# StanislavParovoy/VQ-VAE-WaveNet

Hardware: AMD Instinct MI355X
Metric: training audio-samples/sec (higher is better)
Workload: dtype f32 via fp16x3 (storage and accumulation fp32; the engine's contraction operands are each fp32 value split into two fp16 planes = 22-23 significand bits, products h1h1 + h1h2 + h2h1 on the fp16 MFMA, device-side range guards -- forward, input and weight gradients of the residual stack, of the 1x1 co; 1 GPU; VCTK '64' encoder, len=6656 batch=8 per GPU, fp32 (fp16x3 engine), full train step (fwd+bwd+allreduce+Adam+EMA); global_batch=8, seq_len=6656, parallelism=dp1

## Files before the change

vq-vae-wavenet_amd/csrc/gate_f16x3.hip:

```cpp
#include <string.h>

#include <type_traits>

#include "vqw_common.h"

namespace {

typedef _Float16 f16x8 __attribute__((ext_vector_type(8)));
typedef unsigned short u16;

typedef __bf16 bf16x8 __attribute__((ext_vector_type(8)));
__device__ __forceinline__ u16 f16_bits(_Float16 h) { return __builtin_bit_cast(u16, h); }
__device__ __forceinline__ u16 bf16_bits(float x) { return __builtin_bit_cast(u16, (__bf16)x); }
template <bool BF = false>
__device__ __forceinline__ void split8(const float (&x)[8], uint4& p0, uint4& p1) {
    u16 a[8], b[8];
#pragma unroll
    for (int e = 0; e < 8; ++e) {
        if (BF) { a[e] = bf16_bits(x[e]); b[e] = 0; continue; }
        float xe = x[e];
        asm volatile("" : "+v"(xe));
        const _Float16 h1 = (_Float16)xe;
        a[e] = f16_bits(h1);
        b[e] = f16_bits((_Float16)(xe - (float)h1));
    }
    p0 = make_uint4(a[0] | ((unsigned)a[1] << 16), a[2] | ((unsigned)a[3] << 16), a[4] | ((unsigned)a[5] << 16), a[6] | ((unsigned)a[7] << 16));
    p1 = make_uint4(b[0] | ((unsigned)b[1] << 16), b[2] | ((unsigned)b[3] << 16), b[4] | ((unsigned)b[5] << 16), b[6] | ((unsigned)b[7] << 16));
}

constexpr float F16_MAX = 65504.0f;
__device__ __forceinline__ float dev_scale(const float* p) { return p ? *p : 1.0f; }
__device__ __forceinline__ float inv_scales(float host_inv, const float* sa, const float* sb) {
    return (sa || sb) ? host_inv * __builtin_amdgcn_rcpf(dev_scale(sa) * dev_scale(sb)) : host_inv;
}
__device__ __forceinline__ float wave_max(float v) {
#pragma unroll
    for (int o = 32; o > 0; o >>= 1) v = fmaxf(v, __shfl_xor(v, o, 64));
    return v;
}
__device__ __forceinline__ void guard_report(float m, bool bad, float ps, unsigned* amax, int* flag) {
    if (!amax && !flag) return;
    const float wm = wave_max(m);
    const bool wbad = __any(bad || !(m * ps <= F16_MAX));
    if ((threadIdx.x & 63) == 0) {
        const unsigned bits = __float_as_uint(wm);
        if (amax && bits > __hip_atomic_load(amax, __ATOMIC_RELAXED, __HIP_MEMORY_SCOPE_AGENT)) atomicMax(amax, bits);
        if (flag && wbad) atomicOr(flag, 1);
    }
}

template <bool BF>
__global__ void split_act_kernel(const float* __restrict__ x, uint4* __restrict__ planes, int B, int C, int T, float scale, int kc0, int KC,
                                 const float* __restrict__ scale_dev, unsigned* amax, int* flag, int s2d) {
    const size_t NB = (size_t)B * T;
    const size_t i = (size_t)blockIdx.x * blockDim.x + threadIdx.x;
    const bool live = i < NB * (C / 8);
    const float sc = scale * dev_scale(scale_dev);
    float m = 0.0f;
    bool bad = false;
    if (live) {
        const size_t row = i % NB;
        const int kc = (int)(i / NB);
        const int b = (int)(row / T), t = (int)(row % T);
        float v[8];
#pragma unroll
        for (int e = 0; e < 8; ++e) {
            const float xv = x[((size_t)b * C + kc * 8 + e) * T + t];
            v[e] = xv * sc;
            bad |= !(fabsf(xv) <= 3.0e38f);
            m = fmaxf(m, fabsf(xv));
        }
        uint4 p0, p1;
        split8<BF>(v, p0, p1);
        if (s2d) {
            const size_t NH = NB / 2, r2 = (size_t)b * (T / 2) + t / 2;
            const int kcs = (t & 1) * (C / 8) + kc;
            planes[(size_t)kcs * NH + r2] = p0;
            if (!BF) planes[((size_t)(C / 4) + kcs) * NH + r2] = p1;
        } else {
            planes[(size_t)(kc0 + kc) * NB + row] = p0;
            if (!BF) planes[((size_t)KC + kc0 + kc) * NB + row] = p1;
        }
    }
    if (!amax && !flag) return;
    __shared__ float smax[4];
    __shared__ int sbad[4];
    const float wm = wave_max(m);
    const bool wbad = __any(bad || !(m * sc <= F16_MAX));
    if ((threadIdx.x & 63) == 0) { smax[threadIdx.x >> 6] = wm; sbad[threadIdx.x >> 6] = wbad; }
    __syncthreads();
    if (threadIdx.x == 0) {
        const unsigned bits = __float_as_uint(fmaxf(fmaxf(smax[0], smax[1]), fmaxf(smax[2], smax[3])));
        if (amax && bits > __hip_atomic_load(amax, __ATOMIC_RELAXED, __HIP_MEMORY_SCOPE_AGENT)) atomicMax(amax, bits);
        if (flag && (sbad[0] | sbad[1] | sbad[2] | sbad[3])) atomicOr(flag, 1);
    }
}

__global__ void amax_kernel(const float* __restrict__ x, long rows, int cols, long ld, long mstride, unsigned* amax, int* flag) {
    const float* xb = x + (size_t)blockIdx.y * mstride;
    const size_t n = (size_t)rows * cols;
    float m = 0.0f;
    bool bad = false;
    const size_t tid = (size_t)blockIdx.x * blockDim.x + threadIdx.x, nthr = (size_t)gridDim.x * blockDim.x;
    if (ld == cols && (n & 3) == 0 && (reinterpret_cast<uintptr_t>(xb) & 15u) == 0) {
        const f32x4* x4 = reinterpret_cast<const f32x4*>(xb);
        const size_t n4 = n >> 2;
        auto fold = [&](const f32x4 v) {
#pragma unroll
            for (int e = 0; e < 4; ++e) {
                const float a = fabsf(v[e]);
                bad |= !(a <= 3.0e38f);
                m = fmaxf(m, a);
            }
        };
        size_t i = tid;
        for (; i + 7 * nthr < n4; i += 8 * nthr) {
            f32x4 v[8];
#pragma unroll
            for (int u = 0; u < 8; ++u) v[u] = __builtin_nontemporal_load(x4 + i + u * nthr);
#pragma unroll
            for (int u = 0; u < 8; ++u) fold(v[u]);
        }
        for (; i < n4; i += nthr) fold(__builtin_nontemporal_load(x4 + i));
    } else {
        for (size_t i = tid; i < n; i += nthr) {
            const float v = xb[(i / cols) * ld + (i % cols)];
            bad |= !(fabsf(v) <= 3.0e38f);
            m = fmaxf(m, fabsf(v));
        }
    }
    __shared__ float smax[4];
    __shared__ int sbad[4];
    const float wm = wave_max(m);
    const bool wbad = __any(bad);
    if ((threadIdx.x & 63) == 0) { smax[threadIdx.x >> 6] = wm; sbad[threadIdx.x >> 6] = wbad; }
    __syncthreads();
    if (threadIdx.x == 0) {
        const unsigned bits = __float_as_uint(fmaxf(fmaxf(smax[0], smax[1]), fmaxf(smax[2], smax[3])));
        unsigned* dst = amax + blockIdx.y;
        if (bits > __hip_atomic_load(dst, __ATOMIC_RELAXED, __HIP_MEMORY_SCOPE_AGENT)) atomicMax(dst, bits);
        if (flag && (sbad[0] | sbad[1] | sbad[2] | sbad[3])) atomicOr(flag, 1);
    }
}

__global__ void update_scales_kernel(unsigned* amax, float* scale, int n, int target_exp, int reset, int* flag, const int* skip) {
    const int i = blockIdx.x * blockDim.x + threadIdx.x;
    if (i >= n || (skip && *skip)) return;
    const unsigned b = amax[i];
    if (b >= 0x7f800000u) {
        if (flag) atomicOr(flag, 1);
    } else if (b != 0) {
        int e = (int)(b >> 23) - 127;
        int se = target_exp - 1 - e;
        se = se > 100 ? 100 : (se < -100 ? -100 : se);
        scale[i] = __uint_as_float((unsigned)(se + 127) << 23);
    } else if (scale[i] == 0.0f) {
        scale[i] = 1.0f;
    }
    if (reset) amax[i] = 0;
}

template <bool BF>
__global__ void pack_gate_w_kernel(const float* __restrict__ w, uint4* __restrict__ planes, int ks, int R, int ldw, float scale,
                                   const float* __restrict__ scale_dev, int hb) {
    scale *= dev_scale(scale_dev);
    const int M = 2 * R, KC = ks * R / 8;
    w += (size_t)blockIdx.y * ks * R * ldw;
    planes += (size_t)blockIdx.y * 2 * KC * M;
    const int i = blockIdx.x * blockDim.x + threadIdx.x;
    if (i >= KC * M) return;
    const int mp = i % M, kc = i / M;
    const int mt = mp / hb, ii = mp % hb, hh = hb / 2;
    const int col = ii < hh ? hh * mt + ii : R + hh * mt + (ii - hh);
    const int j = kc / (R / 8), c0 = (kc % (R / 8)) * 8;
    float v[8];
#pragma unroll
    for (int e = 0; e < 8; ++e) v[e] = w[((size_t)j * R + c0 + e) * ldw + col] * scale;
    uint4 p0, p1;
    split8<BF>(v, p0, p1);
    planes[(size_t)kc * M + mp] = p0;
    if (!BF) planes[((size_t)KC + kc) * M + mp] = p1;
}

template <bool BF>
__global__ void pack_w_kernel(const float* __restrict__ w, uint4* __restrict__ planes, int K, int M, int ldw, float scale,
                              const float* __restrict__ scale_dev) {
    scale *= dev_scale(scale_dev);
    const int KC = K / 8;
    w += (size_t)blockIdx.y * K * ldw;
    planes += (size_t)blockIdx.y * 2 * KC * M;
    const int i = blockIdx.x * blockDim.x + threadIdx.x;
    if (i >= KC * M) return;
    const int m = i % M, kc = i / M;
    float v[8];
#pragma unroll
    for (int e = 0; e < 8; ++e) v[e] = w[(size_t)(kc * 8 + e) * ldw + m] * scale;
    uint4 p0, p1;
    split8<BF>(v, p0, p1);
    planes[(size_t)kc * M + m] = p0;
    if (!BF) planes[((size_t)KC + kc) * M + m] = p1;
}

template <bool BF>
__global__ void pack_w_t_kernel(const float* __restrict__ w, uint4* __restrict__ planes, int K, int M, int Kin, int ld_src, long blk_stride,
                                float scale, const float* __restrict__ scale_dev) {
    scale *= dev_scale(scale_dev);
    const int KC = K / 8;
    w += (size_t)blockIdx.y * (K / Kin) * blk_stride;
    planes += (size_t)blockIdx.y * 2 * KC * M;
    const int i = blockIdx.x * blockDim.x + threadIdx.x;
    if (i >= KC * M) return;
    const int m = i % M, kc = i / M, k0 = kc * 8, jb = k0 / Kin, ko = k0 - jb * Kin;
    const float* src = w + (size_t)jb * blk_stride + (size_t)m * ld_src + ko;
    const f32x4 a = *reinterpret_cast<const f32x4*>(src), b = *reinterpret_cast<const f32x4*>(src + 4);
    float v[8];
#pragma unroll
    for (int e = 0; e < 4; ++e) { v[e] = a[e] * scale; v[4 + e] = b[e] * scale; }
    uint4 p0, p1;
    split8<BF>(v, p0, p1);
    planes[(size_t)kc * M + m] = p0;
    if (!BF) planes[((size_t)KC + kc) * M + m] = p1;
}

template <bool BF>
__global__ __launch_bounds__(256) void pack_w_t_tile_kernel(const float* __restrict__ w, uint4* __restrict__ planes, int K, int M, int Kin, int ld_src,
                                                            long blk_stride, float scale, const float* __restrict__ scale_dev) {
    __shared__ uint4 lp[2][8][65];
    scale *= dev_scale(scale_dev);
    const int KC = K / 8, mt = (M + 63) / 64;
    const int m0 = (blockIdx.x % mt) * 64, kc0 = (blockIdx.x / mt) * 8, k0 = kc0 * 8, jb = k0 / Kin, ko0 = k0 - jb * Kin;
    w += (size_t)blockIdx.y * (K / Kin) * blk_stride + (size_t)jb * blk_stride + ko0;
    planes += (size_t)blockIdx.y * 2 * KC * M;
#pragma unroll
    for (int r = 0; r < 2; ++r) {
        const int e = threadIdx.x + 256 * r, mm = e >> 3, kq = e & 7;
        float v[8];
        if (m0 + mm < M) {
            const float* src = w + (size_t)(m0 + mm) * ld_src + kq * 8;
            const f32x4 a = *reinterpret_cast<const f32x4*>(src), b = *reinterpret_cast<const f32x4*>(src + 4);
#pragma unroll
            for (int i = 0; i < 4; ++i) { v[i] = a[i] * scale; v[4 + i] = b[i] * scale; }
        } else {
#pragma unroll
            for (int i = 0; i < 8; ++i) v[i] = 0.0f;
        }
        uint4 p0, p1;
        split8<BF>(v, p0, p1);
        lp[0][kq][mm] = p0;
        if (!BF) lp[1][kq][mm] = p1;
    }
    __syncthreads();
#pragma unroll
    for (int r = 0; r < 2; ++r) {
        const int e = threadIdx.x + 256 * r, kq = e >> 6, mm = e & 63;
        if (m0 + mm >= M) continue;
        planes[(size_t)(kc0 + kq) * M + m0 + mm] = lp[0][kq][mm];
        if (!BF) planes[((size_t)KC + kc0 + kq) * M + m0 + mm] = lp[1][kq][mm];
    }
}

struct GateArgs {
    vqw_f16x3_gate_desc d;
    int NB;
    int ratio;
};
struct OutArgs {
    vqw_f16x3_out_desc d;
    int NB;
};

#ifndef VQW_WG_PAT_A
#define VQW_WG_PAT_A 4
#define VQW_WG_PAT_B 2
#endif

#ifndef VQW_SCONV_64
#define VQW_SCONV_64 1
#endif
#ifndef VQW_SCONV_192
#define VQW_SCONV_192 1
#endif
#ifndef VQW_X3_TAP_MINOR
#define VQW_X3_TAP_MINOR 1
#endif
#ifndef VQW_X3_PAT_MEM
#define VQW_X3_PAT_MEM 1
#define VQW_X3_PAT_ALU 2
#endif
constexpr int NSTG = 4, STG_BYTES = 32 * 1024, PIECES = 8;

struct LoopGeom {
    const void* wp;
    const void* xp;
    int M, Cin, ks, dilation, NB, m_row0, n0, t0;
    int xKC, xkc0;
    int dir, T;
    int wks, tj0, tjstep, toff, tsgn, ts2d;
    int sb, sn;
};

#ifndef VQW_X3_STAGGER
#define VQW_X3_STAGGER 0
#endif
__device__ __forceinline__ void x3_stagger(int n) {
    if (VQW_X3_STAGGER > 0 && ((blockIdx.x >> 8) & 1))
        for (int i = 0; i < n; ++i) __builtin_amdgcn_s_sleep(127);
}
template <int MR> struct X3Shape {
    static constexpr int NSTAGE = MR == 8 ? 4 : 3;
    static constexpr int STAGE_BYTES = (MR * 2 + 16) * 1024;
    static constexpr int LDS_BYTES = NSTAGE * STAGE_BYTES;
    static constexpr int DEPTH = MR == 8 ? 2 : 1;
};
template <bool BF, int MR, bool TAB = false, int DEPTH = X3Shape<MR>::DEPTH>
__device__ __forceinline__ void f16x3_mainloop(f32x16 (&acc)[MR][2], char* smem, const LoopGeom& g, int wv, int lane) {
    constexpr int NP = BF ? 1 : 2;
    constexpr int NA = MR * NP / 4, NBP = 2 * NP;
    if (MR == 4) x3_stagger(VQW_X3_STAGGER);
    constexpr int NSTG_ = DEPTH + 2, STGB = X3Shape<MR>::STAGE_BYTES, BOFF = MR * 2 * 1024;
    const int l31 = lane & 31, lhi = lane >> 5;
    const int KCA = (TAB ? g.wks : g.ks) * g.Cin / 8, KCB = g.Cin / 8, spt = g.Cin / 16;
    const int nsteps = TAB ? g.sn : g.ks * spt;
    const __amdgpu_buffer_rsrc_t ra = vqw_make_rsrc(g.wp, (unsigned)((size_t)NP * KCA * g.M * 16));
    const size_t plane_bytes = (size_t)g.xKC * g.NB * 16, span = (size_t)(g.xKC - g.xkc0) * g.NB * 16;
    const char* xbase = reinterpret_cast<const char*>(g.xp) + (size_t)g.xkc0 * g.NB * 16;
    const unsigned xspan = span < 0x7fffffffu ? (unsigned)span : 0x7fffffffu;
    const __amdgpu_buffer_rsrc_t rb0 = vqw_make_rsrc(xbase, xspan);
    const __amdgpu_buffer_rsrc_t rb1 = vqw_make_rsrc(xbase + (NP > 1 ? plane_bytes : 0), xspan);
    int voffA[NA], pieceA[NA], voffB[NBP], trow[NBP], pieceB[NBP];
#pragma unroll
    for (int i = 0; i < NA; ++i) {
        const int q = wv * NA + i, tile = q / NP, p = q % NP;
        pieceA[i] = tile * 2 + p;
        voffA[i] = ((p * KCA + lhi) * g.M + g.m_row0 + tile * 32 + l31) * 16;
    }
#pragma unroll
    for (int i = 0; i < NBP; ++i) {
        const int q = wv * NBP + i, tile = q / NP, p = q % NP;
        pieceB[i] = tile * 2 + p;
        voffB[i] = (lhi * g.NB + g.n0 + tile * 32 + l31) * 16;
        trow[i] = TAB ? (g.n0 + tile * 32 + l31) % g.T : g.t0 + tile * 32 + l31;
    }
    f32x4 rgA[NA + NBP], rgB[NA + NBP];
    auto rissue = [&](int s_, f32x4 (&rg)[NA + NBP]) {
        const int s = TAB ? s_ + g.sb : s_;
#if VQW_X3_TAP_MINOR
        const int ji = TAB ? s / spt : s % g.ks, kc = TAB ? (s - ji * spt) * 2 : (s / g.ks) * 2;
#else
        const int ji = s / spt, kc = (s - ji * spt) * 2;
#endif
        const int j = TAB ? g.tj0 + g.tjstep * ji : ji;
        const int e_ = TAB ? j - g.toff : 0;
        const int shift = TAB ? g.tsgn * (e_ >> 1) : (g.ks - 1 - j) * g.dilation * (g.dir < 0 ? -1 : 1);
        const int kcx = TAB ? kc + (g.ts2d ? (e_ & 1) * KCB : 0) : kc;
#pragma unroll
        for (int i = 0; i < NA; ++i) rg[i] = vqw_buf_load4(ra, voffA[i] + (j * KCB + kc) * g.M * 16, 0);
#pragma unroll
        for (int i = 0; i < NBP; ++i) {
            const int tr = trow[i] - shift;
            const int vb = (tr >= 0 && tr < g.T) ? voffB[i] + (kcx * g.NB - shift) * 16 : (int)0x80000000;
            rg[NA + i] = vqw_buf_load4((i % NP) ? rb1 : rb0, vb, 0);
        }
    };
    auto rcommit = [&](int s, const f32x4 (&rg)[NA + NBP]) {
        char* dst = smem + (s % NSTG_) * STGB + lane * 16;
#pragma unroll
        for (int i = 0; i < NA; ++i) *reinterpret_cast<f32x4*>(dst + pieceA[i] * 1024) = rg[i];
#pragma unroll
        for (int i = 0; i < NBP; ++i) *reinterpret_cast<f32x4*>(dst + BOFF + pieceB[i] * 1024) = rg[NA + i];
    };
    uint4 fa[MR][NP], fb[2][NP], fbn[2][NP];
    auto read_a = [&](int i, int s) {
        const char* st = smem + (s % NSTG_) * STGB + lane * 16;
#pragma unroll
        for (int p = 0; p < NP; ++p) fa[i][p] = *reinterpret_cast<const uint4*>(st + (i * 2 + p) * 1024);
    };
    auto read_b = [&](uint4 (&b)[2][NP], int s) {
        const char* st = smem + (s % NSTG_) * STGB + lane * 16 + BOFF;
#pragma unroll
        for (int j = 0; j < 2; ++j)
#pragma unroll
            for (int p = 0; p < NP; ++p) b[j][p] = *reinterpret_cast<const uint4*>(st + ((wv * 2 + j) * 2 + p) * 1024);
    };
#pragma unroll
    for (int i = 0; i < MR; ++i)
#pragma unroll
        for (int j = 0; j < 2; ++j)
#pragma unroll
            for (int r = 0; r < 16; ++r) acc[i][j][r] = 0.f;
    auto mfma_rows = [&](int i, const uint4 (&b)[2][NP]) {
        if constexpr (BF) {
#pragma unroll
            for (int q = 0; q < 4; ++q)
                acc[i + (q >> 1)][q & 1] = __builtin_amdgcn_mfma_f32_32x32x16_bf16(__builtin_bit_cast(bf16x8, fa[i + (q >> 1)][0]), __builtin_bit_cast(bf16x8, b[q & 1][0]), acc[i + (q >> 1)][q & 1], 0, 0, 0);
        } else {
#pragma unroll
            for (int term = 0; term < 3; ++term)
#pragma unroll
                for (int q = 0; q < 4; ++q) {
                    const int ii = i + (q >> 1), j = q & 1;
                    const int pa = term == 1 ? 1 : 0, pb = term == 0 ? 1 : 0;
                    acc[ii][j] = __builtin_amdgcn_mfma_f32_32x32x16_f16(__builtin_bit_cast(f16x8, fa[ii][pa]), __builtin_bit_cast(f16x8, b[j][pb]), acc[ii][j], 0, 0, 0);
                }
        }
    };

    rissue(0, rgA); rcommit(0, rgA);
    rissue(1, rgA); rcommit(1, rgA);
    rissue(2, rgA);
    if (DEPTH == 2) rissue(3, rgB);
    asm volatile("s_waitcnt lgkmcnt(0)\n\ts_barrier" ::: "memory");
#pragma unroll
    for (int i = 0; i < MR; ++i) read_a(i, 0);
    read_b(fb, 0);
    auto step = [&](const uint4 (&bc)[2][NP], uint4 (&bn)[2][NP], int s, f32x4 (&rg)[NA + NBP]) {
        asm volatile("s_waitcnt lgkmcnt(0)\n\ts_barrier" ::: "memory");
        const int sn = s + 1 < nsteps ? s + 1 : s;
#ifndef VQW_ABL_NOLDSREAD
        read_b(bn, sn);
#endif
#ifndef VQW_ABL_NOCOMMIT
        rcommit(s + 2, rg);
#endif
#ifndef VQW_ABL_NOGLOBAL
        rissue(s + 2 + DEPTH, rg);
#endif
#pragma unroll
        for (int i = 0; i < MR; i += 2) {
            mfma_rows(i, bc);
#ifndef VQW_ABL_NOLDSREAD
            read_a(i, sn);
            read_a(i + 1, sn);
#endif
        }
#pragma unroll
        for (int k_ = 0; k_ < (BF ? 2 : 6) * MR; ++k_) {
            __builtin_amdgcn_sched_group_barrier(0x008, 1, 0);
            __builtin_amdgcn_sched_group_barrier(0x100 | 0x200 | 0x020, BF ? 2 : VQW_X3_PAT_MEM, 0);
            __builtin_amdgcn_sched_group_barrier(0x002 | 0x004, VQW_X3_PAT_ALU, 0);
        }
    };
    for (int s = 0; s < nsteps; s += 2) {
        step(fb, fbn, s, rgA);
        step(fbn, fb, s + 1, DEPTH == 2 ? rgB : rgA);
    }
}

template <int NG, int DEPTH, typename Ops, typename Req, typename Fin>
__device__ __forceinline__ void x3_epilogue_pipeline(Req&& request, Fin&& finish) {
    static_assert(NG % 2 == 0 && DEPTH >= 0 && DEPTH <= 2, "two named buffers");
    Ops p0, p1;
    request(0, p0);
    if constexpr (DEPTH == 0) {
#pragma unroll
        for (int g = 0; g < NG; ++g) {
            if (g > 0) request(g, p0);
            finish(g, p0);
        }
    } else if constexpr (DEPTH == 2) {
        request(1, p1);
#pragma unroll
        for (int g = 0; g < NG; g += 2) {
            { const Ops c = p0; if (g + 2 < NG) request(g + 2, p0); finish(g, c); }
                { const Ops c = p1; if (g + 3 < NG) request(g + 3, p1); finish(g + 1, c); }
            }
    } else {
#pragma unroll
        for (int g = 0; g < NG; g += 2) {
            request(g + 1, p1);
            finish(g, p0);
                if (g + 2 < NG) request(g + 2, p0);
            finish(g + 1, p1);
            }
    }
}
__device__ __forceinline__ unsigned x3_present(bool present) {
    unsigned m = __builtin_amdgcn_readfirstlane(present ? 0xffffffffu : 0u);
    asm volatile("" : "+s"(m));
    return m;
}
__device__ __forceinline__ float x3_masked(float v, unsigned m) { return __uint_as_float(__float_as_uint(v) & m); }
__device__ __forceinline__ int x3_masked(int i, unsigned m) { return (int)((unsigned)i & m); }
__device__ __forceinline__ void x3_pin_guard(float& gmax, bool& gbad) {
    int gb_i = (int)gbad;
    asm volatile("" : "+v"(gmax), "+v"(gb_i));
    gbad = gb_i != 0;
}
#ifndef VQW_X3_EPI_DEPTH
#define VQW_X3_EPI_DEPTH 2
#endif
#ifndef VQW_X3_GATE_EPI_DEPTH
#define VQW_X3_GATE_EPI_DEPTH 0
#endif
constexpr int EPI_DEPTH = VQW_X3_EPI_DEPTH;

template <bool BF>
__device__ __forceinline__ void store_plane_quad(void* planes, int KC, int NB, int kc, int row, int lhi, const float (&x)[4], float scale = 1.0f) {
    u16 h1[4], h2[4];
#pragma unroll
    for (int e = 0; e < 4; ++e) {
        const float xs = x[e] * scale;
        if (BF) { h1[e] = bf16_bits(xs); h2[e] = 0; continue; }
        const _Float16 a = (_Float16)xs;
        h1[e] = f16_bits(a);
        h2[e] = f16_bits((_Float16)(xs - (float)a));
    }
    char* base = reinterpret_cast<char*>(planes) + ((size_t)kc * NB + row) * 16 + lhi * 8;
    *reinterpret_cast<uint2*>(base) = make_uint2(h1[0] | ((unsigned)h1[1] << 16), h1[2] | ((unsigned)h1[3] << 16));
    if (!BF) *reinterpret_cast<uint2*>(base + (size_t)KC * NB * 16) = make_uint2(h2[0] | ((unsigned)h2[1] << 16), h2[2] | ((unsigned)h2[3] << 16));
}

template <bool BF, int MR>
__global__ __launch_bounds__(256, MR == 8 ? 1 : 2) void gate_f16x3_kernel(const GateArgs a) {
    extern __shared__ __attribute__((aligned(1024))) char smem[];
    const vqw_f16x3_gate_desc& d = a.d;
    const int tid = threadIdx.x, lane = tid & 63, wv = tid >> 6, l31 = lane & 31, lhi = lane >> 5;
    const int R = d.R, T = d.T;
    constexpr int HB = 32 * MR, HH = HB / 2;
    const int n_mt = R / HH;
    const int bid = vqw_xcd_remap(blockIdx.x, gridDim.x);
    const int mt = bid % n_mt, n0 = (bid / n_mt) * 256;
    const int b = n0 / T, t0 = n0 - b * T;
    f32x16 acc[MR][2];
    {
        LoopGeom g;
        g.wp = d.wp; g.xp = d.xp; g.M = 2 * R; g.Cin = R; g.ks = d.ks; g.dilation = d.dilation; g.NB = a.NB;
        g.xKC = R / 8; g.xkc0 = 0; g.dir = 1; g.T = T;
        g.m_row0 = mt * HB; g.n0 = n0; g.t0 = t0;
        f16x3_mainloop<BF, MR>(acc, smem, g, wv, lane);
    }

    const bool hb = d.bias != nullptr, hc = d.cond != nullptr;
    const float* bp = hb ? d.bias : reinterpret_cast<const float*>(d.wp);
    const float* cb = hc ? d.cond + (size_t)b * d.cond_bstride : reinterpret_cast<const float*>(d.wp);
    const int tcol = t0 + 64 * wv + l31;
    const int tz0 = (t0 + 64 * wv) / a.ratio, tz1 = (t0 + 64 * wv + 32) / a.ratio;
    const float winv = inv_scales(d.w_scale_inv, d.x_scale, d.w_scale);
    const unsigned mb = x3_present(hb), mc = x3_present(hc);
    struct Ops { float bf[4], bg[4], f0[4], f1[4], g0[4], g1[4]; };
    auto epilogue = [&](auto step_c) {
        constexpr bool STEP = decltype(step_c)::value;
        const bool s0 = STEP ? false : d.save0 != nullptr, s1 = STEP ? true : d.save1 != nullptr;
        const bool w0 = STEP ? false : d.out0 != nullptr, wp_ = STEP ? true : d.out_planes != nullptr;
        auto request = [&](int g, Ops& o) {
            const int i = g >> 2, v4 = g & 3;
            const int c0 = HH * mt + 32 * i + 8 * v4 + 4 * lhi;
#pragma unroll
            for (int e = 0; e < 4; ++e) {
                o.bf[e] = bp[x3_masked(c0 + e, mb)]; o.bg[e] = bp[x3_masked(R + c0 + e, mb)];
                const int cf = (c0 + e) * d.cond_T, cg = (R + c0 + e) * d.cond_T;
                o.f0[e] = cb[x3_masked(cf + tz0, mc)]; o.f1[e] = cb[x3_masked(cf + tz1, mc)];
                o.g0[e] = cb[x3_masked(cg + tz0, mc)]; o.g1[e] = cb[x3_masked(cg + tz1, mc)];
            }
        };
        auto finish = [&](int g, const Ops& o) {
            const int i = g >> 2, v4 = g & 3;
            const int c0 = HH * mt + 32 * i + 8 * v4 + 4 * lhi;
            float addf[4][2], addg[4][2];
#pragma unroll
            for (int e = 0; e < 4; ++e) {
                const float bfv = o.bf[e], bgv = o.bg[e], f0 = o.f0[e], f1 = o.f1[e], g0 = o.g0[e], g1 = o.g1[e];
                addf[e][0] = x3_masked(bfv, mb) + x3_masked(f0, mc); addf[e][1] = x3_masked(bfv, mb) + x3_masked(f1, mc);
                addg[e][0] = x3_masked(bgv, mb) + x3_masked(g0, mc); addg[e][1] = x3_masked(bgv, mb) + x3_masked(g1, mc);
            }
            const size_t off = ((size_t)b * R + c0) * T + tcol;
            float* po = (w0 ? d.out0 : d.save1) + off;
            float* p0 = s0 ? d.save0 + off : po;
            float* p1 = s1 ? d.save1 + off : po;
            float gq[2][4];
#pragma unroll
            for (int e = 0; e < 4; ++e)
#pragma unroll
                for (int j = 0; j < 2; ++j) {
                    const float xf = acc[i][j][v4 * 4 + e] * winv + addf[e][j];
                    const float xg = acc[i + MR / 2][j][v4 * 4 + e] * winv + addg[e][j];
                    const float th = 1.0f - 2.0f * __builtin_amdgcn_rcpf(__expf(2.0f * xf) + 1.0f);
                    const float sg = __builtin_amdgcn_rcpf(1.0f + __expf(-xg));
                    const int o_ = e * T + 32 * j;
                    gq[j][e] = th * sg;
                    if constexpr (STEP) asm volatile("" : "+v"(gq[j][e]));
                    if (s0) p0[o_] = th;
                    if (s1) p1[o_] = sg;
                    if (w0) po[o_] = gq[j][e];
                }
            if (wp_) {
#pragma unroll
                for (int j = 0; j < 2; ++j)
                    store_plane_quad<BF>(d.out_planes, d.out_planes_KC > 0 ? d.out_planes_KC : R / 8, a.NB, d.out_planes_kc0 + (HH / 8) * mt + 4 * i + v4,
                                     n0 + 64 * wv + 32 * j + l31, lhi, gq[j]);
            }
        };
        x3_epilogue_pipeline<MR * 2, VQW_X3_GATE_EPI_DEPTH, Ops>(request, finish);
    };
    if (!d.out0 && !d.save0 && d.save1 && d.out_planes) epilogue(std::true_type{});
    else epilogue(std::false_type{});
}

template <bool BF, int MR>
__global__ __launch_bounds__(256, MR == 8 ? 1 : 2) void out_f16x3_kernel(const OutArgs a) {
    extern __shared__ __attribute__((aligned(1024))) char smem[];
    const vqw_f16x3_out_desc& d = a.d;
    const int tid = threadIdx.x, lane = tid & 63, wv = tid >> 6, l31 = lane & 31, lhi = lane >> 5;
    const int R = d.R, S = d.S, T = d.T, M = S + R;
    const int Cin = d.Cin > 0 ? d.Cin : R;
    constexpr int HB = 32 * MR;
    const int n_mt = M / HB;
    const int bid = vqw_xcd_remap(blockIdx.x, gridDim.x);
    const int mt = bid % n_mt, n0 = (bid / n_mt) * 256;
    const int b = n0 / T, t0 = n0 - b * T;
    f32x16 acc[MR][2];
    {
        LoopGeom g;
        g.wp = d.wp; g.xp = d.xp; g.M = M; g.Cin = Cin; g.ks = d.ks > 0 ? d.ks : 1; g.dilation = d.dilation > 0 ? d.dilation : 1; g.NB = a.NB;
        g.xKC = d.xp_KC > 0 ? d.xp_KC : Cin / 8; g.xkc0 = d.xp_kc0; g.dir = d.dir < 0 ? -1 : 1; g.T = T;
        g.m_row0 = mt * HB; g.n0 = n0; g.t0 = t0;
        f16x3_mainloop<BF, MR>(acc, smem, g, wv, lane);
    }
    const bool is_skip = mt * HB < S;
    const bool hb = d.bias != nullptr;
    const float* bp = hb ? d.bias : reinterpret_cast<const float*>(d.wp);
    const int tcol = t0 + 64 * wv + l31;
    const float winv = inv_scales(d.w_scale_inv, d.x_scale, d.w_scale);
    const float ps = (d.plane_scale > 0.0f ? d.plane_scale : 1.0f) * dev_scale(d.out_scale);
    const bool hin = is_skip || d.net_in != nullptr;
    const unsigned mb = x3_present(hb), min_ = x3_present(hin);
    const float* in_base = is_skip ? d.skip : (d.net_in ? d.net_in : d.net_out);
    float* out_base = is_skip ? d.skip : d.net_out;
    const int nrows = is_skip ? S : R, mrow0 = is_skip ? 0 : S;
    struct Ops { float bq[4], old[2][4]; };
    auto epilogue = [&](auto pl_c) {
        constexpr bool PL = decltype(pl_c)::value;
        float gmax = 0.0f;
        bool gbad = false;
        auto offset = [&](int g, int& m0) {
            const int i = g >> 2, v4 = g & 3;
            m0 = mt * HB + 32 * i + 8 * v4 + 4 * lhi;
            return ((size_t)b * nrows + (m0 - mrow0)) * T + tcol;
        };
        auto request = [&](int g, Ops& o) {
            int m0;
            const size_t off = offset(g, m0);
            const float* pin = in_base + off;
#pragma unroll
            for (int e = 0; e < 4; ++e) {
                o.bq[e] = bp[x3_masked(m0 + e, mb)];
#pragma unroll
                for (int j = 0; j < 2; ++j) o.old[j][e] = pin[e * T + 32 * j];
            }
        };
        auto finish = [&](int g, const Ops& o) {
            const int i = g >> 2, v4 = g & 3;
            int m0;
            const size_t off = offset(g, m0);
            float* pout = out_base + off;
            float bq[4], old[2][4], nq[2][4];
#pragma unroll
            for (int e = 0; e < 4; ++e) {
                const float bv = o.bq[e];
                bq[e] = x3_masked(bv, mb);
#pragma unroll
                for (int j = 0; j < 2; ++j) { const float ov = o.old[j][e]; old[j][e] = x3_masked(ov, min_); }
            }
#pragma unroll
            for (int e = 0; e < 4; ++e)
#pragma unroll
                for (int j = 0; j < 2; ++j) {
                    nq[j][e] = old[j][e] + (acc[i][j][v4 * 4 + e] * winv + bq[e]);
                    pout[e * T + 32 * j] = nq[j][e];
                }
            if constexpr (PL) {
#pragma unroll
                for (int j = 0; j < 2; ++j) {
#pragma unroll
                    for (int e = 0; e < 4; ++e) { gmax = fmaxf(gmax, fabsf(nq[j][e])); gbad |= !(fabsf(nq[j][e]) <= 3.0e38f); }
                    store_plane_quad<BF>(d.net_out_planes, d.planes_KC > 0 ? d.planes_KC : R / 8, a.NB, d.planes_kc0 + (m0 - S) / 8,
                                     n0 + 64 * wv + 32 * j + l31, lhi, nq[j], ps);
                }
                x3_pin_guard(gmax, gbad);
            }
        };
        x3_epilogue_pipeline<MR * 4, EPI_DEPTH, Ops>(request, finish);
        if constexpr (PL) guard_report(gmax, gbad, ps, d.out_amax, d.flag);
    };
    if (!is_skip && d.net_out_planes) epilogue(std::true_type{});
    else epilogue(std::false_type{});
}

template <int MR, bool BF = false>
__global__ __launch_bounds__(256, MR == 8 ? 1 : 2) void head_f16x3_kernel(const OutArgs a) {
    extern __shared__ __attribute__((aligned(1024))) char smem[];
    const vqw_f16x3_out_desc& d = a.d;
    const int tid = threadIdx.x, lane = tid & 63, wv = tid >> 6, l31 = lane & 31, lhi = lane >> 5;
    const int M = d.R, T = d.T;
    constexpr int HB = 32 * MR;
    const int n_mt = M / HB;
    const int bid = vqw_xcd_remap(blockIdx.x, gridDim.x);
    const int mt = bid % n_mt, n0 = (bid / n_mt) * 256;
    const int b = n0 / T, t0 = n0 - b * T;
    f32x16 acc[MR][2];
    {
        LoopGeom g;
        g.wp = d.wp; g.xp = d.xp; g.M = M; g.Cin = d.Cin; g.ks = 1; g.dilation = 1; g.NB = a.NB;
        g.xKC = d.xp_KC > 0 ? d.xp_KC : d.Cin / 8; g.xkc0 = d.xp_kc0; g.dir = 1; g.T = T;
        g.m_row0 = mt * HB; g.n0 = n0; g.t0 = t0;
        f16x3_mainloop<BF, MR>(acc, smem, g, wv, lane);
    }
    const bool hb = d.bias != nullptr, hc = d.cond != nullptr, hin = d.net_in != nullptr, hm = d.aux0 != nullptr;
    const bool relu_planes = (d.flags & 1) != 0;
    const float* bp = hb ? d.bias : reinterpret_cast<const float*>(d.wp);
    const float* cb = hc ? d.cond + (size_t)b * d.cond_bstride : reinterpret_cast<const float*>(d.wp);
    const int ratio = hc ? T / d.cond_T : 1;
    const int tz[2] = {(t0 + 64 * wv) / ratio, (t0 + 64 * wv + 32) / ratio};
    const int tcol = t0 + 64 * wv + l31;
    const float winv = inv_scales(d.w_scale_inv, d.x_scale, d.w_scale);
    const float ps = (d.plane_scale > 0.0f ? d.plane_scale : 1.0f) * dev_scale(d.out_scale);
    const int PKC = d.planes_KC > 0 ? d.planes_KC : M / 8;
    const unsigned mb = x3_present(hb), mc = x3_present(hc), min_ = x3_present(hin), mnm = x3_present(!hm);
    const float* in_base = hin ? d.net_in : d.net_out;
    const float* mask_base = hm ? d.aux0 : d.net_out;
    struct Ops { float bv[4], c0[4], c1[4], old[2][4], mv[2][4]; };
    auto epilogue = [&](auto pl_c) {
        constexpr bool PL = decltype(pl_c)::value;
        float gmax = 0.0f;
        bool gbad = false;
        auto request = [&](int g, Ops& o) {
            const int i = g >> 2, v4 = g & 3;
            const int m0 = mt * HB + 32 * i + 8 * v4 + 4 * lhi;
            const size_t off = ((size_t)b * M + m0) * T + tcol;
            const float* pin = in_base + off;
            const float* pm = mask_base + off;
#pragma unroll
            for (int e = 0; e < 4; ++e) {
                o.bv[e] = bp[x3_masked(m0 + e, mb)];
                const int cr = (m0 + e) * d.cond_T;
                o.c0[e] = cb[x3_masked(cr + tz[0], mc)]; o.c1[e] = cb[x3_masked(cr + tz[1], mc)];
#pragma unroll
                for (int j = 0; j < 2; ++j) { o.old[j][e] = pin[e * T + 32 * j]; o.mv[j][e] = pm[e * T + 32 * j]; }
            }
        };
        auto finish = [&](int g, const Ops& o) {
            const int i = g >> 2, v4 = g & 3;
            const int m0 = mt * HB + 32 * i + 8 * v4 + 4 * lhi;
            const size_t off = ((size_t)b * M + m0) * T + tcol;
            float* pout = d.net_out + off;
            float add[4][2], old[2][4], mk[2][4], nq[2][4];
#pragma unroll
            for (int e = 0; e < 4; ++e) {
                const float bv = o.bv[e], c0 = o.c0[e], c1 = o.c1[e];
// ... 1096 lines not shown
```

Baseline: 2.208 million audio-samples/s.

## Stream mainloop tiles global-to-LDS via buffer_load lds DMA instead of register staging

```diff
diff --git a/vq-vae-wavenet_amd/csrc/gate_f16x3.hip b/vq-vae-wavenet_amd/csrc/gate_f16x3.hip
--- a/vq-vae-wavenet_amd/csrc/gate_f16x3.hip
+++ b/vq-vae-wavenet_amd/csrc/gate_f16x3.hip
@@ -259,6 +259,16 @@
     }
 }
 
+__device__ __forceinline__ void x3_dma16(u32x4 rsrc, unsigned lds_dst, int voff) {
+    unsigned keep;
+    asm volatile("s_mov_b32 %0, m0\n\ts_mov_b32 m0, %1\n\ts_nop 0\n\tbuffer_load_dwordx4 %2, %3, 0 offen lds\n\ts_mov_b32 m0, %0"
+                 : "=&s"(keep) : "s"(lds_dst), "v"(voff), "s"(rsrc) : "memory");
+}
+__device__ __forceinline__ u32x4 x3_rsrc_words(const void* p, unsigned bytes) {
+    const size_t a = reinterpret_cast<size_t>(p);
+    return u32x4{(unsigned)a, (unsigned)(a >> 32) & 0xffffu, bytes, 0x00020000u};
+}
+
 struct GateArgs {
     vqw_f16x3_gate_desc d;
     int NB;
@@ -287,7 +297,7 @@
 #define VQW_X3_PAT_MEM 1
 #define VQW_X3_PAT_ALU 2
 #endif
-constexpr int NSTG = 4, STG_BYTES = 32 * 1024, PIECES = 8;
+constexpr int NSTG = 4;
 
 struct LoopGeom {
     const void* wp;
@@ -313,7 +323,9 @@
     static constexpr int DEPTH = MR == 8 ? 2 : 1;
 };
 template <bool BF, int MR, bool TAB = false, int DEPTH = X3Shape<MR>::DEPTH>
-__device__ __forceinline__ void f16x3_mainloop(f32x16 (&acc)[MR][2], char* smem, const LoopGeom& g, int wv, int lane) {
+__device__ __forceinline__ void f16x3_mainloop(f32x16 (&acc)[MR][2], char* smem, const LoopGeom& g, int wv_, int lane_) {
+    int wv = wv_, lane = lane_;
+    asm volatile("" : "+v"(wv), "+v"(lane));
     constexpr int NP = BF ? 1 : 2;
     constexpr int NA = MR * NP / 4, NBP = 2 * NP;
     if (MR == 4) x3_stagger(VQW_X3_STAGGER);
@@ -321,28 +333,28 @@
     const int l31 = lane & 31, lhi = lane >> 5;
     const int KCA = (TAB ? g.wks : g.ks) * g.Cin / 8, KCB = g.Cin / 8, spt = g.Cin / 16;
     const int nsteps = TAB ? g.sn : g.ks * spt;
-    const __amdgpu_buffer_rsrc_t ra = vqw_make_rsrc(g.wp, (unsigned)((size_t)NP * KCA * g.M * 16));
     const size_t plane_bytes = (size_t)g.xKC * g.NB * 16, span = (size_t)(g.xKC - g.xkc0) * g.NB * 16;
     const char* xbase = reinterpret_cast<const char*>(g.xp) + (size_t)g.xkc0 * g.NB * 16;
     const unsigned xspan = span < 0x7fffffffu ? (unsigned)span : 0x7fffffffu;
-    const __amdgpu_buffer_rsrc_t rb0 = vqw_make_rsrc(xbase, xspan);
-    const __amdgpu_buffer_rsrc_t rb1 = vqw_make_rsrc(xbase + (NP > 1 ? plane_bytes : 0), xspan);
-    int voffA[NA], pieceA[NA], voffB[NBP], trow[NBP], pieceB[NBP];
+    int voffA[NA], voffB[NBP], trow[NBP];
 #pragma unroll
     for (int i = 0; i < NA; ++i) {
         const int q = wv * NA + i, tile = q / NP, p = q % NP;
-        pieceA[i] = tile * 2 + p;
         voffA[i] = ((p * KCA + lhi) * g.M + g.m_row0 + tile * 32 + l31) * 16;
     }
 #pragma unroll
     for (int i = 0; i < NBP; ++i) {
-        const int q = wv * NBP + i, tile = q / NP, p = q % NP;
-        pieceB[i] = tile * 2 + p;
+        const int tile = (wv * NBP + i) / NP;
         voffB[i] = (lhi * g.NB + g.n0 + tile * 32 + l31) * 16;
         trow[i] = TAB ? (g.n0 + tile * 32 + l31) % g.T : g.t0 + tile * 32 + l31;
     }
-    f32x4 rgA[NA + NBP], rgB[NA + NBP];
-    auto rissue = [&](int s_, f32x4 (&rg)[NA + NBP]) {
+    constexpr int P = NA + NBP;
+    const u32x4 ra = x3_rsrc_words(g.wp, (unsigned)((size_t)NP * KCA * g.M * 16));
+    const u32x4 rb0 = x3_rsrc_words(xbase, xspan), rb1 = x3_rsrc_words(xbase + (NP > 1 ? plane_bytes : 0), xspan);
+    const unsigned lds0 = (unsigned)(size_t)(__attribute__((address_space(3))) char*)smem;
+    const int wvu = __builtin_amdgcn_readfirstlane(wv);
+    struct StageReq { int woff, xoff, shift; unsigned dst; };
+    auto stage_req = [&](int s_) {
         const int s = TAB ? s_ + g.sb : s_;
 #if VQW_X3_TAP_MINOR
         const int ji = TAB ? s / spt : s % g.ks, kc = TAB ? (s - ji * spt) * 2 : (s / g.ks) * 2;
@@ -353,21 +365,19 @@
         const int e_ = TAB ? j - g.toff : 0;
         const int shift = TAB ? g.tsgn * (e_ >> 1) : (g.ks - 1 - j) * g.dilation * (g.dir < 0 ? -1 : 1);
         const int kcx = TAB ? kc + (g.ts2d ? (e_ & 1) * KCB : 0) : kc;
-#pragma unroll
-        for (int i = 0; i < NA; ++i) rg[i] = vqw_buf_load4(ra, voffA[i] + (j * KCB + kc) * g.M * 16, 0);
-#pragma unroll
-        for (int i = 0; i < NBP; ++i) {
-            const int tr = trow[i] - shift;
-            const int vb = (tr >= 0 && tr < g.T) ? voffB[i] + (kcx * g.NB - shift) * 16 : (int)0x80000000;
-            rg[NA + i] = vqw_buf_load4((i % NP) ? rb1 : rb0, vb, 0);
-        }
-    };
-    auto rcommit = [&](int s, const f32x4 (&rg)[NA + NBP]) {
-        char* dst = smem + (s % NSTG_) * STGB + lane * 16;
-#pragma unroll
-        for (int i = 0; i < NA; ++i) *reinterpret_cast<f32x4*>(dst + pieceA[i] * 1024) = rg[i];
-#pragma unroll
-        for (int i = 0; i < NBP; ++i) *reinterpret_cast<f32x4*>(dst + BOFF + pieceB[i] * 1024) = rg[NA + i];
+        return StageReq{(j * KCB + kc) * g.M * 16, (kcx * g.NB - shift) * 16, shift, lds0 + (unsigned)((s_ % NSTG_) * STGB)};
+    };
+    auto dma_piece = [&](const StageReq& r, int q) {
+#ifndef VQW_ABL_NODMA
+        if (q < NA) {
+            const int w = wvu * NA + q;
+            x3_dma16(ra, r.dst + (unsigned)((w / NP * 2 + w % NP) * 1024), voffA[q] + r.woff);
+        } else {
+            const int i = q - NA, w = wvu * NBP + i, tr = trow[i] - r.shift;
+            const int vb = (tr >= 0 && tr < g.T) ? voffB[i] + r.xoff : (int)0x80000000;
+            x3_dma16((i % NP) ? rb1 : rb0, r.dst + (unsigned)(BOFF + (w / NP * 2 + w % NP) * 1024), vb);
+        }
+#endif
     };
     uint4 fa[MR][NP], fb[2][NP], fbn[2][NP];
     auto read_a = [&](int i, int s) {
@@ -405,26 +415,28 @@
         }
     };
 
-    rissue(0, rgA); rcommit(0, rgA);
-    rissue(1, rgA); rcommit(1, rgA);
-    rissue(2, rgA);
-    if (DEPTH == 2) rissue(3, rgB);
-    asm volatile("s_waitcnt lgkmcnt(0)\n\ts_barrier" ::: "memory");
+    auto wait_barrier = [&](auto n_c) {
+        constexpr int N = decltype(n_c)::value;
+        static_assert(N < 64, "vmcnt is a 6-bit counter");
+        asm volatile("s_waitcnt vmcnt(%0) lgkmcnt(0)\n\ts_barrier" :: "n"(N) : "memory");
+    };
+#pragma unroll
+    for (int s = 0; s < NSTG_; ++s) {
+        const StageReq r = stage_req(s);
+#pragma unroll
+        for (int q = 0; q < P; ++q) dma_piece(r, q);
+    }
+    wait_barrier(std::integral_constant<int, (NSTG_ - 1) * P>{});
 #pragma unroll
     for (int i = 0; i < MR; ++i) read_a(i, 0);
     read_b(fb, 0);
-    auto step = [&](const uint4 (&bc)[2][NP], uint4 (&bn)[2][NP], int s, f32x4 (&rg)[NA + NBP]) {
-        asm volatile("s_waitcnt lgkmcnt(0)\n\ts_barrier" ::: "memory");
+    auto step = [&](const uint4 (&bc)[2][NP], uint4 (&bn)[2][NP], int s) {
+        wait_barrier(std::integral_constant<int, DEPTH * P>{});
         const int sn = s + 1 < nsteps ? s + 1 : s;
 #ifndef VQW_ABL_NOLDSREAD
         read_b(bn, sn);
 #endif
-#ifndef VQW_ABL_NOCOMMIT
-        rcommit(s + 2, rg);
-#endif
-#ifndef VQW_ABL_NOGLOBAL
-        rissue(s + 2 + DEPTH, rg);
-#endif
+        const StageReq r = stage_req(s + NSTG_);
 #pragma unroll
         for (int i = 0; i < MR; i += 2) {
             mfma_rows(i, bc);
@@ -432,6 +444,8 @@
             read_a(i, sn);
             read_a(i + 1, sn);
 #endif
+#pragma unroll
+            for (int q = P * (i / 2) / (MR / 2); q < P * (i / 2 + 1) / (MR / 2); ++q) dma_piece(r, q);
         }
 #pragma unroll
         for (int k_ = 0; k_ < (BF ? 2 : 6) * MR; ++k_) {
@@ -441,9 +455,10 @@
         }
     };
     for (int s = 0; s < nsteps; s += 2) {
-        step(fb, fbn, s, rgA);
-        step(fbn, fb, s + 1, DEPTH == 2 ? rgB : rgA);
-    }
+        step(fb, fbn, s);
+        step(fbn, fb, s + 1);
+    }
+    asm volatile("s_waitcnt vmcnt(0)" ::: "memory");
 }
 
 template <int NG, int DEPTH, typename Ops, typename Req, typename Fin>
```

Result: faster. 2.241 million audio-samples/s, median of 6 (+1.5%).
